# YaoFANGUK/video-subtitle-remover

Measured on AMD Instinct MI355X. Metric: inpainted frames/sec @1080p (STTN, 5-frame window), higher is better.
Workload: dtype f32; 1 GPU; 1080p synthetic clip, --inpaint-mode sttn-auto, 50-frame chunks resident in HBM, neighbor stride 5 / refs every 10 (BASELINE.json metric; model cost is resolution-independent); chunk_frames=50, parallelism=chunk-parallel x1, weights=synthetic variance-preserving (no checkpoint in the reference mount)

## Files before the change

### include/vsr_hip.h

```cpp
#ifndef VSR_HIP_H
#define VSR_HIP_H
#include <stdint.h>

#ifdef __cplusplus
extern "C" {
#endif

#define VSR_OK 0
#define VSR_ERR_ARG (-1)
#define VSR_ERR_STATE (-2)
#define VSR_ERR_HIP (-3)
#define VSR_ERR_NOGPU (-4)

#define VSR_VARIANT_STTN_AUTO 0
#define VSR_VARIANT_STTN_DET 1

typedef struct vsr_sttn vsr_sttn_t;
typedef struct vsr_plan vsr_plan_t;

int vsr_version(void);
const char* vsr_last_error(void);
int vsr_device_count(void);

int vsr_sttn_create(int variant, vsr_sttn_t** out);
// ... 43 lines not shown

double vsr_sttn_flops(vsr_sttn_t* h, int L);
double vsr_sttn_flops_reference(vsr_sttn_t* h, int L);

int vsr_sttn_timing(vsr_sttn_t* h, int enable);
int vsr_sttn_timing_get(vsr_sttn_t* h, const char* tag_prefix, double* total_ms, int32_t* launches, double* flops);
int vsr_sttn_timing_reset(vsr_sttn_t* h);

#define VSR_GG_KC 32
enum { VSR_BMODE_NK = 0, VSR_BMODE_KN = 1 };
enum { VSR_ACT_NONE = 0, VSR_ACT_LRELU02 = 1, VSR_ACT_RELU = 2, VSR_ACT_LRELU01 = 3,
       VSR_ACT_OUT_SPLIT = 0x100,
       VSR_ACT_POST_RELU = 0x200,
       VSR_ACT_ROW_MAX = 0x400, VSR_ACT_A_EXP = 0x800 };
#define VSR_VARIANT_A_EXP 0x100
#define VSR_VARIANT_NARROW 8
enum { VSR_TILE_128x128 = 0, VSR_TILE_256x32 = 1, VSR_TILE_256x64 = 2, VSR_TILE_128x64 = 3,
       VSR_TILE_256x128 = 4,
       VSR_TILE_256x256 = 5   };

typedef struct GGProblem {
    const float* A;
    const float* B;
    float* C;
    const float* bias;
    const float* R;
    const int32_t* rowA;
    const int32_t* colA;
    const int32_t* rowB;
    const int32_t* colB;
// ... 250 lines not shown
int64_t vsr_plan_consts(const vsr_plan_t* p, float* out, int64_t capacity);
void vsr_plan_destroy(vsr_plan_t* p);
int vsr_plan_num_buffers(const vsr_plan_t* p);
int64_t vsr_plan_buffer_elems(const vsr_plan_t* p, int buf);
int vsr_plan_num_tables(const vsr_plan_t* p);
int64_t vsr_plan_table_len(const vsr_plan_t* p, int t);
int vsr_plan_table_copy(const vsr_plan_t* p, int t, int32_t* out);
int vsr_plan_num_ops(const vsr_plan_t* p);
int vsr_plan_op(const vsr_plan_t* p, int i, VsrOpInfo* out);
int vsr_plan_op_lane(const vsr_plan_t* p, int i);
int vsr_plan_op_gemm(const vsr_plan_t* p, int i, int j, VsrGemmInfo* out);
int vsr_plan_op_softmax(const vsr_plan_t* p, int i, int j, VsrSoftmaxInfo* out);
int vsr_plan_counts(const vsr_plan_t* p, int32_t* counts);
double vsr_plan_flops(const vsr_plan_t* p);
double vsr_plan_flops_executed(const vsr_plan_t* p);

#ifdef __cplusplus
}
#endif
#endif
```

### video-subtitle-remover_amd/_lib.py

```python
import ctypes as C
import os

_HERE = os.path.dirname(os.path.abspath(__file__))
LIB_PATH = os.path.join(_HERE, "lib", "libvsr_hip.so")

VSR_OK, VSR_ERR_ARG, VSR_ERR_STATE, VSR_ERR_HIP, VSR_ERR_NOGPU = 0, -1, -2, -3, -4
VARIANT = {"auto": 0, "det": 1}
BMODE_NK, BMODE_KN = 0, 1
ACT_NONE, ACT_LRELU02 = 0, 1
TILE_128x128, TILE_256x32, TILE_256x64, TILE_128x64 = 0, 1, 2, 3
TILE_256x128, TILE_256x256 = 4, 5
TILE_DIMS = {TILE_128x128: (128, 128), TILE_256x32: (256, 32), TILE_256x64: (256, 64), TILE_128x64: (128, 64), TILE_256x128: (256, 128), TILE_256x256: (256, 256)}


class VsrError(RuntimeError):
    def __init__(self, code, msg):
        super().__init__(f"libvsr_hip error {code}: {msg}")
        self.code = code


class GGProblem(C.Structure):
    _fields_ = [("A", C.c_void_p), ("B", C.c_void_p), ("C", C.c_void_p), ("bias", C.c_void_p), ("R", C.c_void_p),
                ("rowA", C.c_void_p), ("colA", C.c_void_p), ("rowB", C.c_void_p), ("colB", C.c_void_p),
                ("rowC", C.c_void_p), ("colC", C.c_void_p), ("rowR", C.c_void_p),
# ... 192 lines not shown
    "vsr_plan_consts": (_L, [_P, _P, _L]),
    "vsr_plan_destroy": (None, [_P]),
    "vsr_plan_num_buffers": (_I, [_P]),
    "vsr_plan_buffer_elems": (_L, [_P, _I]),
    "vsr_plan_num_tables": (_I, [_P]),
    "vsr_plan_table_len": (_L, [_P, _I]),
    "vsr_plan_table_copy": (_I, [_P, _I, _P]),
    "vsr_plan_num_ops": (_I, [_P]),
    "vsr_plan_op": (_I, [_P, _I, C.POINTER(VsrOpInfo)]),
    "vsr_plan_op_lane": (_I, [_P, _I]),
    "vsr_plan_op_gemm": (_I, [_P, _I, _I, C.POINTER(VsrGemmInfo)]),
    "vsr_plan_op_softmax": (_I, [_P, _I, _I, C.POINTER(VsrSoftmaxInfo)]),
    "vsr_plan_counts": (_I, [_P, _P]),
    "vsr_plan_flops": (_D, [_P]),
    "vsr_plan_flops_executed": (_D, [_P]),
    "vsr_switch_state": (_I, [C.c_char_p]),
    "vsr_flow_timing": (_I, [_I]),
    "vsr_flow_timing_reset": (_I, []),
    "vsr_flow_timing_get": (_I, [C.c_char_p, C.POINTER(C.c_double), C.POINTER(C.c_int64), C.POINTER(C.c_double)]),
    "vsr_flow_timing_keys": (C.c_int64, [_P, C.c_int64]),
}

if not os.path.exists(LIB_PATH):
    raise ImportError(
        f"{LIB_PATH} is missing: build the HIP extension first (__graft_entry__.build() or "
        f"`make -C {os.path.join(_HERE, 'csrc')}`); this package has no CPU fallback")

import torch

from . import switches
# ... 18 lines not shown
```

### video-subtitle-remover_amd/csrc/gather_gemm.hip

```cpp
#include <hip/hip_runtime.h>
#include <stdlib.h>
#include "gather_gemm.h"

typedef float f32x4 __attribute__((ext_vector_type(4)));
typedef float f32x16 __attribute__((ext_vector_type(16)));

#define GG_LD 36

typedef const float __attribute__((address_space(1)))* gcf32;
typedef float __attribute__((address_space(1)))* gf32;
typedef const int32_t __attribute__((address_space(1)))* gci32;
typedef const f32x4 __attribute__((address_space(1)))* gcf32x4;
typedef const int32_t __attribute__((address_space(4)))* cci32;

__device__ __forceinline__ unsigned int f32_ordered(float f)
{
    const unsigned int b = __float_as_uint(f);
    return (b & 0x80000000u) ? ~b : (b | 0x80000000u);
}
__device__ __forceinline__ float f32_from_ordered(unsigned int e)
{
    return __uint_as_float((e & 0x80000000u) ? (e & 0x7fffffffu) : ~e);
}

// ... 391 lines not shown
                                            variant == 6, stream);                                              \
        } else if (queue && variant == 7) {                                                                     \
            static const int resident = resident_blocks(gather_gemm_f32_v4<BM, BN, WM, WN, MODE, true>);       \
            const int g = totalBlocks < resident ? totalBlocks : resident;                                     \
            hipLaunchKernelGGL((gather_gemm_f32_v4<BM, BN, WM, WN, MODE, true>), dim3(g), block, 0, stream,    \
                               d_probs, nprobs, totalBlocks, queue, nQueues == 8 ? 8 : 1, rangeFlag);          \
        } else if (queue && variant == 4) {                                                                     \
            static const int resident = resident_blocks(gather_gemm_f32_v4<BM, BN, WM, WN, MODE, false>);      \
            const int g = totalBlocks < resident ? totalBlocks : resident;                                     \
            hipLaunchKernelGGL((gather_gemm_f32_v4<BM, BN, WM, WN, MODE, false>), dim3(g), block, 0, stream,   \
                               d_probs, nprobs, totalBlocks, queue, nQueues == 8 ? 8 : 1, rangeFlag);          \
        } else if (queue) {                                                                                     \
            static const int resident = resident_blocks(gather_gemm_f32_v3<BM, BN, WM, WN, MODE>);             \
            const int g = totalBlocks < resident ? totalBlocks : resident;                                     \
            hipLaunchKernelGGL((gather_gemm_f32_v3<BM, BN, WM, WN, MODE>), dim3(g), block, 0, stream, d_probs, \
                               nprobs, totalBlocks, queue, ((nQueues & 0xff) == 8 ? 8 : 1) | (nQueues & 0x100));    \
        } else {                                                                                                \
            hipLaunchKernelGGL((gather_gemm_f32<BM, BN, WM, WN, MODE>), dim3(totalBlocks), block, 0, stream,   \
                               d_probs, nprobs);                                                               \
        }                                                                                                       \
    } while (0)

extern "C" int vsr_launch_gather_gemm_dev(const GGProblem* d_probs, int nprobs, int totalBlocks, int tileCfg,
                                          int bmode, unsigned int* queue, int variant, int nQueues,
                                          unsigned int* rangeFlag, void* stream_)
{
    hipStream_t stream = (hipStream_t)stream_;
    if (totalBlocks <= 0) return 0;
    dim3 block(256);
    if (variant & VSR_VARIANT_A_EXP) {
        if ((variant & 0xff) != 1 || bmode != VSR_BMODE_KN) return -1;
        if (tileCfg == VSR_TILE_128x64) hipLaunchKernelGGL((gather_gemm_f32_aexp<128, 64, 2, 2>), dim3(totalBlocks), block, 0, stream, d_probs, nprobs);
        else if (tileCfg == VSR_TILE_128x128) hipLaunchKernelGGL((gather_gemm_f32_aexp<128, 128, 2, 2>), dim3(totalBlocks), block, 0, stream, d_probs, nprobs);
        else return -1;
        return hipGetLastError() == hipSuccess ? 0 : VSR_ERR_HIP;
    }
    if (variant <= 1) queue = nullptr;
    if (tileCfg == VSR_TILE_256x128) {
        if (bmode != VSR_BMODE_NK || variant != 6 || !queue) return -1;
        launch_v6_st<256, 128, 4, 2, 3>(d_probs, nprobs, totalBlocks, queue, nQueues == 8 ? 8 : 1, rangeFlag, stream);
        return hipGetLastError() == hipSuccess ? 0 : VSR_ERR_HIP;
    }
    if (tileCfg == VSR_TILE_256x256) {
        if (bmode != VSR_BMODE_NK || (variant != 6 && variant != 5) || !queue) return -1;
        launch_v7(d_probs, nprobs, totalBlocks, queue, rangeFlag, variant == 6, stream);
        return hipGetLastError() == hipSuccess ? 0 : VSR_ERR_HIP;
    }
    if (tileCfg == VSR_TILE_128x128 && bmode == VSR_BMODE_NK) GG_LAUNCH(128, 128, 2, 2, VSR_BMODE_NK);
// ... 24 lines not shown
```

### video-subtitle-remover_amd/csrc/gather_gemm_pvx.h

```cpp
#pragma once

template <int BM, int BN, int WM, int WN>
__global__ void __launch_bounds__(256)
gather_gemm_f32_aexp(const GGProblem* __restrict__ probs, int nprobs)
{
    constexpr int WTM = BM / WM, WTN = BN / WN;
    constexpr int MI = WTM / 32, NI = WTN / 32;
    constexpr int A_IT = BM / 32;
    constexpr int LDB_KN = BN + 4;
    constexpr int TPR = BN / 4;
    constexpr int RPP = 256 / TPR;
    constexpr int B_IT = 32 / RPP;
    static_assert(WM * WN == 4, "4 waves");

    __shared__ __attribute__((aligned(16))) float smem[BM * GG_LD + 32 * LDB_KN];
    float* As = smem;
    float* Bs = smem + BM * GG_LD;

    const int bid = blockIdx.x;
    int pi = 0;
    for (int lo_ = 0, hi_ = nprobs - 1; lo_ < hi_;) {
        const int mid_ = (lo_ + hi_ + 1) >> 1;
        if (bid >= probs[mid_].tileStart) lo_ = mid_; else hi_ = mid_ - 1;
        pi = lo_;
// ... 20 lines not shown
    if (kcEnd > nchunksTotal) kcEnd = nchunksTotal;

    const gcf32 A = (gcf32)P->A;
    const gcf32 B = (gcf32)P->B;
    const gci32 rowA = (gci32)P->rowA;
    const cci32 colA = (cci32)P->colA;
    const gci32 rowB = (gci32)P->rowB;
    const cci32 colB = (cci32)P->colB;
    const bool aexp = (P->act & VSR_ACT_A_EXP) != 0;

    const int tid = threadIdx.x;
    const int lane = tid & 63;
    const int wave = __builtin_amdgcn_readfirstlane(tid >> 6);
    const int wm = wave / WN, wn = wave % WN;
    const int l31 = lane & 31, hi = lane >> 5;

    const int s_r = tid >> 3, s_q = tid & 7;
    int aoff[A_IT];
    float mrow[A_IT], lsum[A_IT];
#pragma unroll
    for (int it = 0; it < A_IT; ++it) {
        aoff[it] = rowA[tm * BM + s_r + 32 * it] + 4 * s_q;
        lsum[it] = 0.f;
        mrow[it] = 0.f;
    }
    if (aexp) {
        const unsigned int __attribute__((address_space(1)))* rmax = (const unsigned int __attribute__((address_space(1)))*)P->bias;
#pragma unroll
        for (int it = 0; it < A_IT; ++it) mrow[it] = f32_from_ordered(rmax[tm * BM + s_r + 32 * it]);
    }
// ... 4 lines not shown

    f32x4 ra[A_IT], rb[B_IT];
    f32x16 acc[MI][NI];
#pragma unroll
    for (int mi = 0; mi < MI; ++mi)
#pragma unroll
        for (int ni = 0; ni < NI; ++ni)
#pragma unroll
            for (int r = 0; r < 16; ++r) acc[mi][ni][r] = 0.f;

    auto load_rowB = [&](int kc, int (&dst)[B_IT]) {
#pragma unroll
        for (int it = 0; it < B_IT; ++it) dst[it] = rowB[kc * VSR_GG_KC + k_r + RPP * it];
    };
    auto load_tile = [&](int kc) {
        const int ca = colA[kc];
#pragma unroll
        for (int it = 0; it < A_IT; ++it) ra[it] = *(gcf32x4)(A + (aoff[it] + ca));
#pragma unroll
        for (int it = 0; it < B_IT; ++it) rb[it] = *(gcf32x4)(B + (boff[it] + bcolKN));
    };
    const bool needSum = aexp && (splitK == 1 || tn == 0);
    auto store_tile = [&]() {
        if (aexp) {
#pragma unroll
            for (int it = 0; it < A_IT; ++it)
#pragma unroll
                for (int j = 0; j < 4; ++j) ra[it][j] = __builtin_amdgcn_exp2f(ra[it][j] - mrow[it]);
            if (needSum) {
#pragma unroll
                for (int it = 0; it < A_IT; ++it) lsum[it] += (ra[it][0] + ra[it][1]) + (ra[it][2] + ra[it][3]);
// ... 11 lines not shown
        for (int g = 0; g < 4; ++g) {
            f32x4 af[MI], bf[NI];
#pragma unroll
            for (int mi = 0; mi < MI; ++mi)
                af[mi] = *reinterpret_cast<const f32x4*>(&As[(wm * WTM + mi * 32 + l31) * GG_LD + 8 * g + 4 * hi]);
#pragma unroll
            for (int ni = 0; ni < NI; ++ni)
#pragma unroll
                for (int j = 0; j < 4; ++j)
                    bf[ni][j] = Bs[(8 * g + 4 * hi + j) * LDB_KN + wn * WTN + ni * 32 + l31];
#pragma unroll
            for (int j = 0; j < 4; ++j)
#pragma unroll
                for (int mi = 0; mi < MI; ++mi)
#pragma unroll
                    for (int ni = 0; ni < NI; ++ni)
                        acc[mi][ni] = __builtin_amdgcn_mfma_f32_32x32x2f32(af[mi][j], bf[ni][j], acc[mi][ni], 0, 0, 0);
        }
    };

    if (kcBeg < kcEnd) {
        load_rowB(kcBeg, boff);
        if (kcBeg + 1 < kcEnd) load_rowB(kcBeg + 1, boffNext);
        load_tile(kcBeg);
        store_tile();
        __syncthreads();
        for (int kc = kcBeg; kc < kcEnd; ++kc) {
            const bool hasNext = (kc + 1 < kcEnd);
            if (hasNext) {
#pragma unroll
                for (int it = 0; it < B_IT; ++it) boff[it] = boffNext[it];
                load_tile(kc + 1);
                if (kc + 2 < kcEnd) load_rowB(kc + 2, boffNext);
            }
            compute_tile();
            __syncthreads();
            if (hasNext) store_tile();
            __syncthreads();
        }
    }

    float* lrow = smem;
    const bool partial = (splitK > 1);
    if (aexp) {
#pragma unroll
        for (int it = 0; it < A_IT; ++it) {
            float s = lsum[it];
            s += __shfl_xor(s, 1, 64);
            s += __shfl_xor(s, 2, 64);
            s += __shfl_xor(s, 4, 64);
// ... 1 lines not shown
        }
        __syncthreads();
        if (partial && tn == 0 && tid < BM)
            const_cast<float*>(P->R)[(int64_t)split * tilesM * BM + tm * BM + tid] = lrow[tid];
    }

    const float alpha = P->alpha;
    const int act = P->act & 0xff;
    const bool postRelu = (P->act & VSR_ACT_POST_RELU) != 0;
    const gcf32 bias = (partial || aexp) ? (gcf32) nullptr : (gcf32)P->bias;
    const gcf32 R = (partial || aexp) ? (gcf32) nullptr : (gcf32)P->R;
    const gci32 rowC = (gci32)P->rowC;
    const cci32 colC = (cci32)P->colC;
    const gci32 rowR = (gci32)P->rowR;
    const gf32 C = (gf32)(P->C + (partial ? (int64_t)split * P->splitStride : (int64_t)0));

    int ccol[NI];
    float bv[NI];
    bool nok[NI];
#pragma unroll
    for (int ni = 0; ni < NI; ++ni) {
        const int n0 = tn * BN + wn * WTN + ni * 32;
        ccol[ni] = colC[n0 / VSR_GG_KC] + l31;
        nok[ni] = (n0 + l31) < N;
        bv[ni] = (bias != nullptr && nok[ni]) ? bias[n0 + l31] : 0.f;
    }
#pragma unroll
    for (int mi = 0; mi < MI; ++mi) {
#pragma unroll
        for (int r = 0; r < 16; ++r) {
// ... 20 lines not shown
```

### video-subtitle-remover_amd/csrc/gather_gemm_v3.h

```cpp
#pragma once
#include <type_traits>

typedef __attribute__((address_space(3))) void* lds_vptr;

__device__ __forceinline__ void glds16(gcf32 src, lds_vptr dst)
{
#if defined(__HIP_DEVICE_COMPILE__)
    __builtin_amdgcn_global_load_lds(src, dst, 16, 0, 0);
#else
    (void)src; (void)dst;
#endif
}

#ifdef GG_ABLATE
__device__ unsigned long long gg_trace[1024 * 256];
#define GG_STAMP()                                                                     \
    if constexpr (GG_ABL(64)) {                                                        \
        if (tid == 0 && blockIdx.x < 1024 && tr_ < 256)                                \
            gg_trace[blockIdx.x * 256 + tr_] = __builtin_readcyclecounter();           \
        ++tr_;                                                                         \
    }
#define GG_PH(k)                                                                       \
    if constexpr (GG_ABL(32)) {                                                        \
        const unsigned long long now_ = __builtin_readcyclecounter();                  \
// ... 27 lines not shown
    constexpr int BS_FLOATS = BN * 32;
    constexpr int BUF_FLOATS = AS_FLOATS + BS_FLOATS;
    constexpr int CB_BIAS = 2 * BM, CB_COLC = 2 * BM + BN, CB_CTL = CB_COLC + BN / 32;
    constexpr int CB_WORDS = (CB_CTL + 16 + 3) / 4 * 4;
    constexpr int RT_IT = (CB_WORDS + 255) / 256;
    enum { CW_M = 0, CW_N, CW_ALPHA, CW_ACT, CW_SPLITK, CW_CLO, CW_CHI, CW_RLO, CW_RHI, CW_HASBIAS };
    constexpr bool PIPE = (BMODE == VSR_BMODE_NK) && !GG_ABL(2048);
    static_assert(WM * WN == 4, "4 waves");

    __shared__ __attribute__((aligned(16))) float smem[2 * BUF_FLOATS + 2 * CB_WORDS + BM * WN + 4];
    int* rowTabs = reinterpret_cast<int*>(smem + 2 * BUF_FLOATS);
    float* scr = smem + 2 * BUF_FLOATS + 2 * CB_WORDS;
    volatile int* nextTile = reinterpret_cast<volatile int*>(smem + 2 * BUF_FLOATS + 2 * CB_WORDS + BM * WN);

    const bool swizzle = (nQueues & 0x100) != 0;
    nQueues &= 0xff;
    const int tid = threadIdx.x;
    const int lane = tid & 63;
    const int wave = __builtin_amdgcn_readfirstlane(tid >> 6);
    const int wm = wave / WN, wn = wave % WN;
    const int l31 = lane & 31, hi = lane >> 5;
    const int s_r = tid >> 3, s_q = tid & 7;
    const int k_r = tid / TPR, k_q = tid % TPR;
    const int srcSwz = ((s_q ^ ((s_r >> 1) & 7)) << 2);
    int rdOff[4];
#pragma unroll
    for (int g_ = 0; g_ < 4; ++g_) rdOff[g_] = (((2 * g_ + hi) ^ ((l31 >> 1) & 7)) << 2);

    int qFirst = 0;
    const int qShift = nQueues == 8 ? 3 : 0;
// ... 101 lines not shown
        } else {
            const gci32 colB = (gci32)q.P->colB;
            tb.bcolKN = colB[(q.tn * BN) / VSR_GG_KC + (k_q >> 3)];
        }
        fetchCols(q, q.kcBeg, tb.vcolA, tb.vcolB);
        fetchCols(q, q.kcBeg + 64, tb.vcolAn, tb.vcolBn);
        const gci32 rowCt = (gci32)gg_uniform_ptr(q.P->rowC);
        const gci32 rowRt = (gci32)gg_uniform_ptr(q.P->rowR);
        const int pact = q.P->act, psplitK = q.P->splitK, pN = q.P->N;
        const bool partial = psplitK > 1;
        const bool hasR = (q.P->R != nullptr) && !partial && !(pact & VSR_ACT_ROW_MAX);
        const gcf32 biasp = partial ? (gcf32) nullptr : (gcf32)gg_uniform_ptr(q.P->bias);
        const cci32 colCp = (cci32)gg_uniform_ptr(q.P->colC);
        const unsigned long long cptr = reinterpret_cast<unsigned long long>(q.P->C + (partial ? (int64_t)q.split * q.P->splitStride : (int64_t)0));
        const unsigned long long rptr = reinterpret_cast<unsigned long long>(q.P->R);
#pragma unroll
        for (int k = 0; k < RT_IT; ++k) {
            const int i = tid + 256 * k;
            int v = 0;
            if (i < BM) v = rowCt[q.tm * BM + i];
            else if (i < 2 * BM) { if (hasR) v = rowRt[q.tm * BM + i - BM]; }
            else if (i < CB_COLC) { const int n = q.tn * BN + i - CB_BIAS; if (biasp != nullptr && n < pN) v = __float_as_int(biasp[n]); }
            else if (i < CB_CTL) v = colCp[(q.tn * BN) / VSR_GG_KC + i - CB_COLC];
            else {
                const int w = i - CB_CTL;
                v = w == CW_M ? q.P->M : w == CW_N ? pN : w == CW_ALPHA ? __float_as_int(q.P->alpha) : w == CW_ACT ? pact : w == CW_SPLITK ? psplitK
                  : w == CW_CLO ? (int)(unsigned)cptr : w == CW_CHI ? (int)(unsigned)(cptr >> 32) : w == CW_RLO ? (int)(unsigned)rptr
                  : w == CW_RHI ? (int)(unsigned)(rptr >> 32) : w == CW_HASBIAS ? (biasp != nullptr ? 1 : 0) : 0;
            }
            tb.rt[k] = v;
        }
    };
    auto make_rows = [&](const Tab& tb, Rows& rw) __attribute__((always_inline)) {
// ... 183 lines not shown

        const int kcEndU = __builtin_amdgcn_readfirstlane(g.kcEnd);
        const int kcBegU = __builtin_amdgcn_readfirstlane(g.kcBeg);
        if (!ready) {
            if (kcBegU < kcEndU) {
                if constexpr (BMODE == VSR_BMODE_KN) {
                    load_rowB_KN(kcBegU, boff);
                    if (kcBegU + 1 < kcEndU) load_rowB_KN(kcBegU + 1, boffNext);
                }
                dma_tile(kcBegU, B0_{});
            }
            __syncthreads();
        }
        __builtin_amdgcn_s_setprio(0);
        GG_STAMP()

        auto chunk = [&](int kc, auto cur, auto nxt, auto modeTag) __attribute__((always_inline)) {
            constexpr int MODE = decltype(modeTag)::value;
#ifdef GG_ABLATE
            if constexpr (GG_ABL(32)) { tl_ = __builtin_readcyclecounter(); ph_[4] += 1; }
#endif
            __builtin_amdgcn_s_setprio(3);
            if constexpr (MODE == 1) {
                if (tid == 0) *nextTile = claim_end();
                published = true;
            }
            if (MODE != 3 && (MODE == 2 || kc + 1 < kcEndU)) {
                if (kc + 1 - colBase >= 64) {
                    colBase += 64;
                    vcolA = vcolAn; vcolB = vcolBn;
// ... 18 lines not shown
            }
            if constexpr (MODE == 3) {
                if (haveN) {
                    Rows rN;
                    make_rows(tN, rN);
                    const int ca = __builtin_amdgcn_readlane(tN.vcolA, 0);
                    const int cb = __builtin_amdgcn_readlane(tN.vcolB, 0);
                    const GGProblem* PN = gg_uniform_ptr(gN.P);
                    dma_pieces(gN, (gcf32)gg_uniform_ptr(PN->A), (gcf32)gg_uniform_ptr(PN->B), rN, boff, 0, ca, cb, nxt);
                    store_rowtab(tN, slot ^ 1);
                }
            }
            __builtin_amdgcn_sched_barrier(0);
            __builtin_amdgcn_s_setprio(0);
            GG_PH(0)
            compute_chunk(cur);
            GG_PH(1)
#ifdef GG_ABLATE
            if constexpr (GG_ABL(32)) { asm volatile("s_waitcnt vmcnt(0)" ::: "memory"); }
#endif
            GG_PH(2)
            if constexpr (!GG_ABL(1)) __syncthreads();
            GG_PH(3)
            GG_STAMP()
        };
        using M0_ = std::integral_constant<int, 0>;
        using M1_ = std::integral_constant<int, 1>;
        using M2_ = std::integral_constant<int, 2>;
        using M3_ = std::integral_constant<int, 3>;
        auto run = [&](auto s0, auto s1) __attribute__((always_inline)) {
            int kc = kcBegU;
// ... 205 lines not shown
```

### video-subtitle-remover_amd/csrc/sttn_engine.hip

```cpp
#include <hip/hip_runtime.h>
#include <algorithm>
#include <math.h>
#include <stdio.h>
#include <stdlib.h>
#include <string.h>
#include <map>
#include <memory>
#include <string>
#include <utility>
#include <vector>
#include "../../include/vsr_hip.h"
#include "elementwise.h"
#include "gather_gemm.h"
#include "sttn_plan.h"

using namespace vsr;

static thread_local std::string g_err;
static int fail(int code, const std::string& msg)
{
    g_err = msg;
    return code;
}
int vsr_internal_fail(int code, const char* msg) { return fail(code, msg); }
// ... 346 lines not shown
{
    if (precision >= 2) return precision == 3 ? 6 : 5;
    if (precision) {
        static const int pv = [] { const char* e = getenv("VSR_SPLIT_PV_VARIANT"); int x = e ? atoi(e) : 4; return (x < 1 || x > 4) ? 4 : x; }();
        return bmode == VSR_BMODE_KN ? pv : 4;
    }
    static const int nk = [] { const char* e = getenv("VSR_GG_VARIANT"); int x = e ? atoi(e) : 3; return (x < 1 || x > 4) ? 3 : x; }();
    static const int kn = [] {
        const char* e = getenv("VSR_PV_VARIANT");
        const char* g = getenv("VSR_GG_VARIANT");
        int x = e ? atoi(e) : ((g && atoi(g) <= 3) ? atoi(g) : 1);
        return (x < 1 || x > 3) ? 1 : x;
    }();
    return bmode == VSR_BMODE_KN ? kn : nk;
}
static bool use_persistent() { return gg_variant(VSR_BMODE_NK) >= 2 || gg_variant(VSR_BMODE_KN) >= 2; }

static bool sttn_thin(int precision, int bmode, const std::vector<GGProblem>& probs, int totalTiles)
{
    static const int mode = [] { const char* e = getenv("VSR_STTN_THIN"); return e ? atoi(e) : 0; }();
    static const int maxTiles = [] { const char* e = getenv("VSR_STTN_THIN_TILES"); return e ? atoi(e) : 768; }();
    static const int maxK = [] { const char* e = getenv("VSR_STTN_THIN_K"); return e ? atoi(e) : 2600; }();
    static const int shortK = [] { const char* e = getenv("VSR_STTN_THIN_SHORT_K"); return e ? atoi(e) : 256; }();
    if (mode == 0 || precision != 0 || bmode != VSR_BMODE_NK || probs.empty() || gg_variant(VSR_BMODE_NK) != 3) return false;
    int K = 0;
    for (const GGProblem& q : probs) {
        if (q.act & VSR_ACT_ROW_MAX) return false;
        K = std::max(K, q.splitK > 1 ? q.chunksPerSplit * VSR_GG_KC : q.K);
    }
    return K <= shortK || (totalTiles <= maxTiles && K <= maxK);
// ... 44 lines not shown
            HIPCHK(hipEventCreate(&tr.b));
            HIPCHK(hipEventRecord(tr.a, stream));
        }
        int rc = 0;
        static const bool qkSplit = [] { const char* e = getenv("VSR_F16_QK_SPLIT"); return e && atoi(e) == 1; }();
        const bool scoresSplit = prec == 3 && qkSplit && od.kind == OP_GEMM && od.tag == "attn.qk";
        switch (od.kind) {
        case OP_GEMM:
            for (const OpDev::Vt& vt : od.vts)
                if (rc == 0) rc = vsr_launch_kn_to_nk_split(vt.B, vt.rowB, vt.colB, vt.K, vt.N, vt.ld, vt.dst, stream);
            if (rc == 0 && od.total7 > 0)
                rc = vsr_launch_gather_gemm_dev((const GGProblem*)od.dDesc7, od.nitems7, od.total7, VSR_TILE_256x256, VSR_BMODE_NK, queue + 8,
                                                (prec == 3 && !scoresSplit) ? 6 : 5, 1, h->dRangeFlag, stream);
            if (rc == 0 && od.total > 0)
                rc = vsr_launch_gather_gemm_dev((const GGProblem*)od.dDesc, od.nitems, od.total, od.tileCfg, od.bmode, queue,
                                                (scoresSplit ? 5 : od.thin ? 1 : gg_variant(od.bmode, prec)) | (od.aexp ? VSR_VARIANT_A_EXP : 0), od.nQueues,
                                                prec ? h->dRangeFlag : nullptr, stream);
            break;
        case OP_SOFTMAX:
            rc = vsr_launch_softmax_dev((const SMProblem*)od.dDesc, od.nitems, od.total, stream);
            break;
        case OP_NORM_IM2COL:
            rc = vsr_launch_norm_im2col_fmt((const uint8_t*)od.src, od.H, od.W, od.n, (float*)od.dst, od.premask, od.maskU8, od.split, stream);
            break;
        case OP_UPSAMPLE2X:
            rc = vsr_launch_upsample2x_rows((const float*)od.src, od.H, od.W, od.C, od.haloS, (float*)od.dst, od.haloD, od.n, od.split,
                                            od.rowLo, od.rowHi > od.rowLo ? od.rowHi : 2 * od.H, stream);
            break;
        case OP_DECODE_OUT:
            if (od.rowHi > od.rowLo && od.W > 0)
                rc = vsr_launch_decode_out_rows((const float*)od.src, od.ldy, od.pix, od.n, od.tFrameIdx, od.tFirst, (float*)od.dst,
// ... 642 lines not shown
static void tile_dims(int cfg, int& BM, int& BN)
{
    BM = (cfg == VSR_TILE_128x128 || cfg == VSR_TILE_128x64) ? 128 : 256;
    BN = cfg == VSR_TILE_256x256 ? 256 : (cfg == VSR_TILE_128x128 || cfg == VSR_TILE_256x128) ? 128 : ((cfg == VSR_TILE_256x64 || cfg == VSR_TILE_128x64) ? 64 : 32);
}

static int run_gather_gemm_variant(const GGProblem* probs, int nprobs, int tile_cfg, int bmode, int variant, void* stream_);

int vsr_run_gather_gemm(const GGProblem* probs, int nprobs, int tile_cfg, int bmode, void* stream_)
{
    return run_gather_gemm_variant(probs, nprobs, tile_cfg, bmode, gg_variant(bmode), stream_);
}

int vsr_run_gather_gemm_variant(const GGProblem* probs, int nprobs, int tile_cfg, int bmode, int variant, void* stream_)
{
    if (variant != (1 | VSR_VARIANT_A_EXP) && variant != VSR_VARIANT_NARROW && (variant < 1 || variant > 6))
        return fail(VSR_ERR_ARG, "kernel variant must be 1..6, VSR_VARIANT_NARROW or 1 | VSR_VARIANT_A_EXP");
    return run_gather_gemm_variant(probs, nprobs, tile_cfg, bmode, variant, stream_);
}

struct vsr_gemm_plan {
    GGProblem* d = nullptr;
    unsigned int* queue = nullptr;
    int nprobs = 0, total = 0, tileCfg = 0, bmode = 0, variant = 3, nQueues = 8, device = 0;
};

int vsr_gemm_plan_create(const GGProblem* probs, int nprobs, int tile_cfg, int bmode, int variant, vsr_gemm_plan_t** out)
{
    if (!probs || nprobs <= 0 || !out) return fail(VSR_ERR_ARG, "bad argument");
    if (variant < 1 || variant > 4) return fail(VSR_ERR_ARG, "kernel variant must be 1..4 (fp32 tensors)");
    if (vsr_device_count() <= 0) return fail(VSR_ERR_NOGPU, "no HIP device; there is no CPU fallback");
    std::vector<GGProblem> hp(probs, probs + nprobs);
// ... 241 lines not shown
    const Op& op = p->plan->ops[i];
    if (op.kind != OP_SOFTMAX || j < 0 || j >= (int)op.softmax.size()) return fail(VSR_ERR_ARG, "bad softmax item");
    const SoftmaxItem& s = op.softmax[j];
    o->bufS = s.bufS; o->bufP = s.bufP; o->offS = s.offS; o->offP = s.offP; o->splitStride = s.splitStride;
    o->M = s.M; o->N = s.N; o->ldS = s.ldS; o->ldP = s.ldP; o->nsplit = s.nsplit; o->scale = s.scale;
    return 0;
}
int vsr_plan_counts(const vsr_plan_t* p, int32_t* counts)
{
    if (!p || !counts) return fail(VSR_ERR_ARG, "bad argument");
    memcpy(counts, p->plan->compCount.data(), p->plan->compCount.size() * sizeof(int32_t));
    return 0;
}
double vsr_plan_flops(const vsr_plan_t* p) { return p ? p->plan->flops : -1.0; }
double vsr_plan_flops_executed(const vsr_plan_t* p) { return !p ? -1.0 : (p->plan->flopsExecuted >= 0 ? p->plan->flopsExecuted : p->plan->flops); }

}
```

### video-subtitle-remover_amd/csrc/sttn_plan.cpp

```cpp
#include "sttn_plan.h"
#include "gather_gemm.h"
#include <algorithm>
#include <assert.h>
#include <math.h>
#include <stdexcept>
#include <stdlib.h>

namespace vsr {

static int envInt(const char* name, int dflt)
{
    const char* v = getenv(name);
    return (v && *v) ? atoi(v) : dflt;
}

const Tuning& Tuning::get(int precision)
{
    static const Tuning t[2] = {
        [] {
            Tuning x;
            x.convTile = envInt("VSR_CONV_TILE", VSR_TILE_128x64);
            if (x.convTile == VSR_TILE_256x128) x.convTile = VSR_TILE_128x64;
            x.qkTile = envInt("VSR_QK_TILE", VSR_TILE_128x64);
            x.qkvTile = envInt("VSR_QKV_TILE", x.convTile);
// ... 1012 lines not shown
        if (neighbors.back() < nCtx) continue;
        lane_ = nwindows % lanes;
        const size_t first = ops.size();
        if (firstWindowOp < 0) firstWindowOp = (int)first;
        buildWindow(neighbors, refs, visits);
        for (size_t i = first; i < ops.size(); ++i) ops[i].lane = lane_;
    }
    lane_ = 0;
    compCount = visits;
    refFlops = flops + trimmedFlops_;
    flopsExecuted = 0;
    for (const Op& op : ops) flopsExecuted += op.flopsExecuted >= 0 ? op.flopsExecuted : op.flops;
    if (nCtx > 0) refFlops = Plan(model, L_, precision_, 1, decLo_, decHi_, decXLo_, decXHi_).refFlops;
}

void cv2_linear_tables(int ssize, int dsize, bool clampX, std::vector<int32_t>& ofs, std::vector<int16_t>& icoef,
                       std::vector<float>& fcoef)
{
    const double inv_scale = (double)dsize / (double)ssize;
    const double scale = 1.0 / inv_scale;
    ofs.resize(dsize);
    icoef.resize(2 * (size_t)dsize);
    fcoef.resize(2 * (size_t)dsize);
    for (int d = 0; d < dsize; ++d) {
        float f = (float)((d + 0.5) * scale - 0.5);
        int s = (int)floorf(f);
        f -= (float)s;
        if (clampX) {
            if (s < 0) { f = 0.f; s = 0; }
            if (s >= ssize - 1) { f = 0.f; s = ssize - 1; }
// ... 18 lines not shown
```

### video-subtitle-remover_amd/csrc/sttn_plan.h

```cpp
#pragma once
#include <stdint.h>
#include <map>
#include <string>
#include <vector>

namespace vsr {

struct Geometry {
    int variant;
    int modelW, modelH;
    int featW, featH;
    int channels;
    int blocks;
    int nscales;
    int patchW[4], patchH[4];
    int neighborStride;
    int refLength;
    static Geometry make(int variant);
};

struct Tuning {
    int convTile;
    int qkTile;
    int qkvTile;
// ... 109 lines not shown
};

constexpr int BUF_PLAN_CONST = -2;

struct PlanIR {
    std::vector<int64_t> bufElems;
    std::vector<float> consts;
    std::vector<std::vector<int32_t>> tables;
    std::vector<Op> ops;
    std::vector<int32_t> compCount;
    double flops = 0;
    double flopsExecuted = -1;
    double refFlops = 0;
    virtual ~PlanIR() {}
};

class PlanBuilder : public PlanIR {
protected:
    std::map<std::string, int> tableKey_;
    int table(const std::string& key, std::vector<int32_t>&& v);
    int tRowsAct(const Act& a, const std::vector<int>& ids, int oh, int ow, int stride, int padTo, int64_t add);
    int tRowsActRect(const Act& a, const std::vector<int>& ids, int ylo, int yhi, int xlo, int xhi, int padTo);
    int tColsConvHW(const Act& a, int kh, int kw, int dil, int c0 = 0, int cin = -1);
    int tColsConv(const Act& a, int ksz, int dil) { return tColsConvHW(a, ksz, ksz, dil); }
    int tColsConvTaps(const Act& a, int dil, unsigned taps);
    int tColsWeightTaps(int cin, unsigned taps);
    int tRowsLinear(int count, int ld, int padTo);
    int tColsLinear(int nchunks, int padTo);
    void need(int buf, int64_t elems);
};
// ... 45 lines not shown
```

Baseline: 223.8 frames/s.

## Skip MFMA work for fully padded waves and add lean PV epilogue

Adds a pad-skip mode, enabled by default, in which waves whose sub-tile lies wholly outside M or N skip the MFMA compute in both the persistent v3 kernel and the A-exp PV kernel. The A-exp kernel gains a LEAN variant. It raises the launch-bounds occupancy hint, broadcasts colA indices from a per-lane register via readlane instead of reloading them, swaps the MFMA operand order, and uses a vectorized float4 epilogue for full aligned tiles. Env vars and variant bits keep the legacy paths reachable, and a helper reports issued FLOPs with and without pad skipping. The aim is to cut wasted matrix work on padded tiles and scalar epilogue stores, at the cost of register pressure and a changed accumulator layout.

```diff
diff --git a/include/vsr_hip.h b/include/vsr_hip.h
--- a/include/vsr_hip.h
+++ b/include/vsr_hip.h
@@ -81,6 +81,8 @@
        VSR_ACT_POST_RELU = 0x200,
        VSR_ACT_ROW_MAX = 0x400, VSR_ACT_A_EXP = 0x800 };
 #define VSR_VARIANT_A_EXP 0x100
+#define VSR_VARIANT_PV_LEGACY 0x200
+#define VSR_VARIANT_NO_PAD_SKIP 0x400
 #define VSR_VARIANT_NARROW 8
 enum { VSR_TILE_128x128 = 0, VSR_TILE_256x32 = 1, VSR_TILE_256x64 = 2, VSR_TILE_128x64 = 3,
        VSR_TILE_256x128 = 4,
@@ -361,6 +363,7 @@
 int vsr_plan_counts(const vsr_plan_t* p, int32_t* counts);
 double vsr_plan_flops(const vsr_plan_t* p);
 double vsr_plan_flops_executed(const vsr_plan_t* p);
+double vsr_plan_flops_issued(const vsr_plan_t* p, int pad_skip);
 
 #ifdef __cplusplus
 }
diff --git a/video-subtitle-remover_amd/_lib.py b/video-subtitle-remover_amd/_lib.py
--- a/video-subtitle-remover_amd/_lib.py
+++ b/video-subtitle-remover_amd/_lib.py
@@ -230,6 +230,7 @@
     "vsr_plan_counts": (_I, [_P, _P]),
     "vsr_plan_flops": (_D, [_P]),
     "vsr_plan_flops_executed": (_D, [_P]),
+    "vsr_plan_flops_issued": (_D, [_P, _I]),
     "vsr_switch_state": (_I, [C.c_char_p]),
     "vsr_flow_timing": (_I, [_I]),
     "vsr_flow_timing_reset": (_I, []),
diff --git a/video-subtitle-remover_amd/csrc/gather_gemm.hip b/video-subtitle-remover_amd/csrc/gather_gemm.hip
--- a/video-subtitle-remover_amd/csrc/gather_gemm.hip
+++ b/video-subtitle-remover_amd/csrc/gather_gemm.hip
@@ -429,7 +429,7 @@
             static const int resident = resident_blocks(gather_gemm_f32_v3<BM, BN, WM, WN, MODE>);             \
             const int g = totalBlocks < resident ? totalBlocks : resident;                                     \
             hipLaunchKernelGGL((gather_gemm_f32_v3<BM, BN, WM, WN, MODE>), dim3(g), block, 0, stream, d_probs, \
-                               nprobs, totalBlocks, queue, ((nQueues & 0xff) == 8 ? 8 : 1) | (nQueues & 0x100));    \
+                               nprobs, totalBlocks, queue, ((nQueues & 0xff) == 8 ? 8 : 1) | (nQueues & 0x100) | (padSkip ? 0x200 : 0)); \
         } else {                                                                                                \
             hipLaunchKernelGGL((gather_gemm_f32<BM, BN, WM, WN, MODE>), dim3(totalBlocks), block, 0, stream,   \
                                d_probs, nprobs);                                                               \
@@ -443,10 +443,17 @@
     hipStream_t stream = (hipStream_t)stream_;
     if (totalBlocks <= 0) return 0;
     dim3 block(256);
+    static const bool padSkipEnv = [] { const char* e = getenv("VSR_PAD_SKIP"); return !(e && atoi(e) == 0); }();
+    const int padSkip = (padSkipEnv && !(variant & VSR_VARIANT_NO_PAD_SKIP)) ? 1 : 0;
+    variant &= ~VSR_VARIANT_NO_PAD_SKIP;
     if (variant & VSR_VARIANT_A_EXP) {
+        const bool legacy = (variant & VSR_VARIANT_PV_LEGACY) != 0;
+        variant &= ~VSR_VARIANT_PV_LEGACY;
         if ((variant & 0xff) != 1 || bmode != VSR_BMODE_KN) return -1;
-        if (tileCfg == VSR_TILE_128x64) hipLaunchKernelGGL((gather_gemm_f32_aexp<128, 64, 2, 2>), dim3(totalBlocks), block, 0, stream, d_probs, nprobs);
-        else if (tileCfg == VSR_TILE_128x128) hipLaunchKernelGGL((gather_gemm_f32_aexp<128, 128, 2, 2>), dim3(totalBlocks), block, 0, stream, d_probs, nprobs);
+        if (tileCfg == VSR_TILE_128x64 && legacy) hipLaunchKernelGGL((gather_gemm_f32_aexp<128, 64, 2, 2, 0>), dim3(totalBlocks), block, 0, stream, d_probs, nprobs, 0);
+        else if (tileCfg == VSR_TILE_128x64) hipLaunchKernelGGL((gather_gemm_f32_aexp<128, 64, 2, 2, 1>), dim3(totalBlocks), block, 0, stream, d_probs, nprobs, padSkip);
+        else if (tileCfg == VSR_TILE_128x128 && legacy) hipLaunchKernelGGL((gather_gemm_f32_aexp<128, 128, 2, 2, 0>), dim3(totalBlocks), block, 0, stream, d_probs, nprobs, 0);
+        else if (tileCfg == VSR_TILE_128x128) hipLaunchKernelGGL((gather_gemm_f32_aexp<128, 128, 2, 2, 1>), dim3(totalBlocks), block, 0, stream, d_probs, nprobs, padSkip);
         else return -1;
         return hipGetLastError() == hipSuccess ? 0 : VSR_ERR_HIP;
     }
diff --git a/video-subtitle-remover_amd/csrc/gather_gemm_pvx.h b/video-subtitle-remover_amd/csrc/gather_gemm_pvx.h
--- a/video-subtitle-remover_amd/csrc/gather_gemm_pvx.h
+++ b/video-subtitle-remover_amd/csrc/gather_gemm_pvx.h
@@ -1,8 +1,8 @@
 #pragma once
 
-template <int BM, int BN, int WM, int WN>
-__global__ void __launch_bounds__(256)
-gather_gemm_f32_aexp(const GGProblem* __restrict__ probs, int nprobs)
+template <int BM, int BN, int WM, int WN, int LEAN = 0>
+__global__ void __launch_bounds__(256, LEAN ? (BN <= 64 ? 4 : 3) : 1)
+gather_gemm_f32_aexp(const GGProblem* __restrict__ probs, int nprobs, int padSkip)
 {
     constexpr int WTM = BM / WM, WTN = BN / WN;
     constexpr int MI = WTM / 32, NI = WTN / 32;
@@ -58,6 +58,14 @@
     const int wave = __builtin_amdgcn_readfirstlane(tid >> 6);
     const int wm = wave / WN, wn = wave % WN;
     const int l31 = lane & 31, hi = lane >> 5;
+    const bool waveOn = !(LEAN && padSkip) || (tm * BM + wm * WTM < M && tn * BN + wn * WTN < N);
+
+    const gci32 colAv = (gci32)P->colA;
+    int vcolA = 0, vcolAn = 0, colBase = kcBeg;
+    auto fetchColA = [&](int base) {
+        const int i = base + lane;
+        return colAv[i < nchunksTotal ? i : nchunksTotal - 1];
+    };
 
     const int s_r = tid >> 3, s_q = tid & 7;
     int aoff[A_IT];
@@ -92,7 +100,8 @@
         for (int it = 0; it < B_IT; ++it) dst[it] = rowB[kc * VSR_GG_KC + k_r + RPP * it];
     };
     auto load_tile = [&](int kc) {
-        const int ca = colA[kc];
+        int ca;
+        if constexpr (LEAN) ca = __builtin_amdgcn_readlane(vcolA, kc - colBase); else ca = colA[kc];
 #pragma unroll
         for (int it = 0; it < A_IT; ++it) ra[it] = *(gcf32x4)(A + (aoff[it] + ca));
 #pragma unroll
@@ -134,12 +143,15 @@
 #pragma unroll
                 for (int mi = 0; mi < MI; ++mi)
 #pragma unroll
-                    for (int ni = 0; ni < NI; ++ni)
-                        acc[mi][ni] = __builtin_amdgcn_mfma_f32_32x32x2f32(af[mi][j], bf[ni][j], acc[mi][ni], 0, 0, 0);
+                    for (int ni = 0; ni < NI; ++ni) {
+                        if constexpr (LEAN) acc[mi][ni] = __builtin_amdgcn_mfma_f32_32x32x2f32(bf[ni][j], af[mi][j], acc[mi][ni], 0, 0, 0);
+                        else acc[mi][ni] = __builtin_amdgcn_mfma_f32_32x32x2f32(af[mi][j], bf[ni][j], acc[mi][ni], 0, 0, 0);
+                    }
         }
     };
 
     if (kcBeg < kcEnd) {
+        if constexpr (LEAN) { vcolA = fetchColA(kcBeg); vcolAn = fetchColA(kcBeg + 64); }
         load_rowB(kcBeg, boff);
         if (kcBeg + 1 < kcEnd) load_rowB(kcBeg + 1, boffNext);
         load_tile(kcBeg);
@@ -150,10 +162,17 @@
             if (hasNext) {
 #pragma unroll
                 for (int it = 0; it < B_IT; ++it) boff[it] = boffNext[it];
+                if constexpr (LEAN) {
+                    if (kc + 1 - colBase >= 64) {
+                        colBase += 64;
+                        vcolA = vcolAn;
+                        vcolAn = fetchColA(colBase + 64);
+                    }
+                }
                 load_tile(kc + 1);
                 if (kc + 2 < kcEnd) load_rowB(kc + 2, boffNext);
             }
-            compute_tile();
+            if (waveOn) compute_tile();
             __syncthreads();
             if (hasNext) store_tile();
             __syncthreads();
@@ -185,6 +204,72 @@
     const cci32 colC = (cci32)P->colC;
     const gci32 rowR = (gci32)P->rowR;
     const gf32 C = (gf32)(P->C + (partial ? (int64_t)split * P->splitStride : (int64_t)0));
+
+    if constexpr (LEAN) {
+        int ccol[NI], ncol[NI];
+#pragma unroll
+        for (int ni = 0; ni < NI; ++ni) {
+            const int n0 = tn * BN + wn * WTN + ni * 32;
+            ccol[ni] = colC[n0 / VSR_GG_KC] + 4 * hi;
+            ncol[ni] = n0 + 4 * hi;
+        }
+        int rc[MI], rr[MI];
+        float inv[MI];
+#pragma unroll
+        for (int mi = 0; mi < MI; ++mi) {
+            const int row = wm * WTM + mi * 32 + l31;
+            rc[mi] = rowC[tm * BM + row];
+            rr[mi] = (R != nullptr) ? rowR[tm * BM + row] : 0;
+            inv[mi] = (aexp && !partial) ? 1.f / lrow[row] : 1.f;
+        }
+        bool vec = (tm * BM + BM <= M) && (tn * BN + BN <= N) && bias == nullptr && R == nullptr && act == VSR_ACT_NONE &&
+                   (reinterpret_cast<unsigned long long>(C) & 15) == 0;
+        {
+            int low = 0;
+#pragma unroll
+            for (int ni = 0; ni < NI; ++ni) low |= ccol[ni];
+#pragma unroll
+            for (int mi = 0; mi < MI; ++mi) low |= rc[mi];
+            vec = vec && __all((low & 3) == 0);
+        }
+        if (vec) {
+            const float bz = 0.f;
+#pragma unroll
+            for (int mi = 0; mi < MI; ++mi)
+#pragma unroll
+                for (int ni = 0; ni < NI; ++ni)
+#pragma unroll
+                    for (int q = 0; q < 4; ++q) {
+                        f32x4 o;
+#pragma unroll
+                        for (int e = 0; e < 4; ++e) o[e] = acc[mi][ni][4 * q + e] * alpha * inv[mi] + bz;
+                        *reinterpret_cast<f32x4 __attribute__((address_space(1)))*>(C + (rc[mi] + ccol[ni] + 8 * q)) = o;
+                    }
+        } else {
+#pragma unroll
+            for (int mi = 0; mi < MI; ++mi) {
+                const bool mok = (tm * BM + wm * WTM + mi * 32 + l31) < M;
+#pragma unroll
+                for (int ni = 0; ni < NI; ++ni)
+#pragma unroll
+                    for (int r = 0; r < 16; ++r) {
+                        const int cofs = (r & 3) + 8 * (r >> 2);
+                        const int n = ncol[ni] + cofs;
+                        const bool ok = mok && n < N;
+                        const float bvn = (bias != nullptr && n < N) ? bias[n] : 0.f;
+                        float v = acc[mi][ni][r] * alpha * inv[mi] + bvn;
+                        if (act == VSR_ACT_LRELU02) v = v > 0.f ? v : 0.2f * v;
+                        else if (act == VSR_ACT_RELU) v = fmaxf(v, 0.f);
+                        else if (act == VSR_ACT_LRELU01) v = v > 0.f ? v : 0.1f * v;
+                        if (ok) {
+                            if (R != nullptr) { v += R[rr[mi] + ccol[ni] + cofs]; if (postRelu) v = fmaxf(v, 0.f); }
+                            C[rc[mi] + ccol[ni] + cofs] = v;
+                        }
+                    }
+            }
+        }
+        return;
+    }
 
     int ccol[NI];
     float bv[NI];
diff --git a/video-subtitle-remover_amd/csrc/gather_gemm_v3.h b/video-subtitle-remover_amd/csrc/gather_gemm_v3.h
--- a/video-subtitle-remover_amd/csrc/gather_gemm_v3.h
+++ b/video-subtitle-remover_amd/csrc/gather_gemm_v3.h
@@ -65,6 +65,7 @@
     volatile int* nextTile = reinterpret_cast<volatile int*>(smem + 2 * BUF_FLOATS + 2 * CB_WORDS + BM * WN);
 
     const bool swizzle = (nQueues & 0x100) != 0;
+    const bool padSkip = (nQueues & 0x200) != 0;
     nQueues &= 0xff;
     const int tid = threadIdx.x;
     const int lane = tid & 63;
@@ -196,9 +197,10 @@
         const cci32 colCp = (cci32)gg_uniform_ptr(q.P->colC);
         const unsigned long long cptr = reinterpret_cast<unsigned long long>(q.P->C + (partial ? (int64_t)q.split * q.P->splitStride : (int64_t)0));
         const unsigned long long rptr = reinterpret_cast<unsigned long long>(q.P->R);
+        const int tidL = wave * 64 + (int)__builtin_amdgcn_mbcnt_hi(~0u, __builtin_amdgcn_mbcnt_lo(~0u, 0u));
 #pragma unroll
         for (int k = 0; k < RT_IT; ++k) {
-            const int i = tid + 256 * k;
+            const int i = tidL + 256 * k;
             int v = 0;
             if (i < BM) v = rowCt[q.tm * BM + i];
             else if (i < 2 * BM) { if (hasR) v = rowRt[q.tm * BM + i - BM]; }
@@ -412,6 +414,10 @@
         }
         __builtin_amdgcn_s_setprio(0);
         GG_STAMP()
+        bool waveOn = true;
+        if (padSkip)
+            waveOn = tm * BM + wm * WTM < __builtin_amdgcn_readfirstlane(rowTab[CB_CTL + CW_M]) &&
+                     tn * BN + wn * WTN < __builtin_amdgcn_readfirstlane(rowTab[CB_CTL + CW_N]);
 
         auto chunk = [&](int kc, auto cur, auto nxt, auto modeTag) __attribute__((always_inline)) {
             constexpr int MODE = decltype(modeTag)::value;
@@ -460,7 +466,7 @@
             __builtin_amdgcn_sched_barrier(0);
             __builtin_amdgcn_s_setprio(0);
             GG_PH(0)
-            compute_chunk(cur);
+            if (waveOn) compute_chunk(cur);
             GG_PH(1)
 #ifdef GG_ABLATE
             if constexpr (GG_ABL(32)) { asm volatile("s_waitcnt vmcnt(0)" ::: "memory"); }
diff --git a/video-subtitle-remover_amd/csrc/sttn_engine.hip b/video-subtitle-remover_amd/csrc/sttn_engine.hip
--- a/video-subtitle-remover_amd/csrc/sttn_engine.hip
+++ b/video-subtitle-remover_amd/csrc/sttn_engine.hip
@@ -384,6 +384,11 @@
     }();
     return bmode == VSR_BMODE_KN ? kn : nk;
 }
+static int pv_aexp_bits()
+{
+    static const int bits = [] { const char* e = getenv("VSR_PV_EPILOGUE"); return VSR_VARIANT_A_EXP | ((e && atoi(e) == 0) ? VSR_VARIANT_PV_LEGACY : 0); }();
+    return bits;
+}
 static bool use_persistent() { return gg_variant(VSR_BMODE_NK) >= 2 || gg_variant(VSR_BMODE_KN) >= 2; }
 
 static bool sttn_thin(int precision, int bmode, const std::vector<GGProblem>& probs, int totalTiles)
@@ -458,7 +463,7 @@
                                                 (prec == 3 && !scoresSplit) ? 6 : 5, 1, h->dRangeFlag, stream);
             if (rc == 0 && od.total > 0)
                 rc = vsr_launch_gather_gemm_dev((const GGProblem*)od.dDesc, od.nitems, od.total, od.tileCfg, od.bmode, queue,
-                                                (scoresSplit ? 5 : od.thin ? 1 : gg_variant(od.bmode, prec)) | (od.aexp ? VSR_VARIANT_A_EXP : 0), od.nQueues,
+                                                (scoresSplit ? 5 : od.thin ? 1 : gg_variant(od.bmode, prec)) | (od.aexp ? pv_aexp_bits() : 0), od.nQueues,
                                                 prec ? h->dRangeFlag : nullptr, stream);
             break;
         case OP_SOFTMAX:
@@ -1131,8 +1136,10 @@
 
 int vsr_run_gather_gemm_variant(const GGProblem* probs, int nprobs, int tile_cfg, int bmode, int variant, void* stream_)
 {
-    if (variant != (1 | VSR_VARIANT_A_EXP) && variant != VSR_VARIANT_NARROW && (variant < 1 || variant > 6))
-        return fail(VSR_ERR_ARG, "kernel variant must be 1..6, VSR_VARIANT_NARROW or 1 | VSR_VARIANT_A_EXP");
+    const int base = variant & ~VSR_VARIANT_NO_PAD_SKIP;
+    const bool padBitOk = base == variant || base == 3 || (base & VSR_VARIANT_A_EXP);
+    if (!padBitOk || (base != (1 | VSR_VARIANT_A_EXP) && base != (1 | VSR_VARIANT_A_EXP | VSR_VARIANT_PV_LEGACY) && base != VSR_VARIANT_NARROW && (base < 1 || base > 6)))
+        return fail(VSR_ERR_ARG, "kernel variant must be 1..6, VSR_VARIANT_NARROW or 1 | VSR_VARIANT_A_EXP [| VSR_VARIANT_PV_LEGACY]; VSR_VARIANT_NO_PAD_SKIP goes with 3 and A_EXP");
     return run_gather_gemm_variant(probs, nprobs, tile_cfg, bmode, variant, stream_);
 }
 
@@ -1404,5 +1411,6 @@
 }
 double vsr_plan_flops(const vsr_plan_t* p) { return p ? p->plan->flops : -1.0; }
 double vsr_plan_flops_executed(const vsr_plan_t* p) { return !p ? -1.0 : (p->plan->flopsExecuted >= 0 ? p->plan->flopsExecuted : p->plan->flops); }
-
-}
+double vsr_plan_flops_issued(const vsr_plan_t* p, int pad_skip) { return !p ? -1.0 : plan_flops_issued(*p->plan, pad_skip != 0); }
+
+}
diff --git a/video-subtitle-remover_amd/csrc/sttn_plan.cpp b/video-subtitle-remover_amd/csrc/sttn_plan.cpp
--- a/video-subtitle-remover_amd/csrc/sttn_plan.cpp
+++ b/video-subtitle-remover_amd/csrc/sttn_plan.cpp
@@ -1050,6 +1050,28 @@
     if (nCtx > 0) refFlops = Plan(model, L_, precision_, 1, decLo_, decHi_, decXLo_, decXHi_).refFlops;
 }
 
+double plan_flops_issued(const PlanIR& plan, bool padSkip)
+{
+    double total = 0;
+    for (const Op& op : plan.ops) {
+        if (op.kind != OP_GEMM) continue;
+        const int c = op.tileCfg;
+        const int BM = (c == VSR_TILE_128x128 || c == VSR_TILE_128x64) ? 128 : 256;
+        const int BN = c == VSR_TILE_256x256 ? 256 : (c == VSR_TILE_128x128 || c == VSR_TILE_256x128) ? 128 : (c == VSR_TILE_256x32 ? 32 : 64);
+        const int WTM = (c == VSR_TILE_256x128 || c == VSR_TILE_256x256) ? 0 : 64;
+        const int WTN = BM == 128 ? BN / 2 : BN;
+        for (const GemmItem& it : op.gemm) {
+            double rows = (double)it.tilesM * BM, cols = (double)it.tilesN * BN;
+            if (padSkip && WTM > 0) {
+                rows = (double)((it.M + WTM - 1) / WTM) * WTM;
+                cols = (double)((it.N + WTN - 1) / WTN) * WTN;
+            }
+            total += 2.0 * rows * cols * it.K;
+        }
+    }
+    return total;
+}
+
 void cv2_linear_tables(int ssize, int dsize, bool clampX, std::vector<int32_t>& ofs, std::vector<int16_t>& icoef,
                        std::vector<float>& fcoef)
 {
diff --git a/video-subtitle-remover_amd/csrc/sttn_plan.h b/video-subtitle-remover_amd/csrc/sttn_plan.h
--- a/video-subtitle-remover_amd/csrc/sttn_plan.h
+++ b/video-subtitle-remover_amd/csrc/sttn_plan.h
@@ -147,6 +147,7 @@
     double refFlops = 0;
     virtual ~PlanIR() {}
 };
+double plan_flops_issued(const PlanIR& plan, bool padSkip);
 
 class PlanBuilder : public PlanIR {
 protected:
```

After: 218.9 frames/s. 2.2% lower.
